# Kamino666/Video-Captioning-Transformer

Measured on AMD Instinct MI355X. Metric: video-caption train samples/sec (whole node), higher is better.
Workload: dtype bf16; 1 GPU; configs[1]: 2 enc + 2 dec layers d=512 ff=2048 H=8 V=30522, synthetic (256,12,512) features -> 20-token captions per GPU, fwd+bwd+Adam, dropout 0.3, SCE alpha 0.5; global_batch=256, per_gpu_batch=256, seq_len=20, frames=12, parallelism=dp1, executor=list

## Files before the change

video-captioning-transformer_amd/csrc/vct_layer_ss.hip:

```cpp
#include "vct_layer_ss_core.h"

namespace vct {

template <bool CROSS, int MT>
__global__ __launch_bounds__(SS_NT, SS_NW / 4) void layer_ss_fwd_kernel(const SsLayerP p) {
  extern __shared__ __attribute__((aligned(16))) unsigned char smem[];
  const int tid0 = threadIdx.x, lane0 = tid0 & 63;
  const int wave = __builtin_amdgcn_readfirstlane(tid0 >> 6);
  const int b = blockIdx.x, L = p.L;
  const long grow0 = (long)b * L;
  bf16_t* R0 = reinterpret_cast<bf16_t*>(smem + SS_R0);
  bf16_t* R1A = reinterpret_cast<bf16_t*>(smem + SS_R1A);
  bf16_t* R1B = reinterpret_cast<bf16_t*>(smem + SS_R1B);
  bf16_t* R1C = reinterpret_cast<bf16_t*>(smem + SS_R1C);
  bf16_t* RMp = reinterpret_cast<bf16_t*>(smem + SS_RM);
  float* red = reinterpret_cast<float*>(smem + SS_RED);
  float* b1s = reinterpret_cast<float*>(smem + SS_B1);

  WStream ws;
  ws.p = p.wpk + (long)wave * SS_WSTR + lane0 * 8;
  ws.last = ws.p + (long)(p.nchunks - 1) * SS_CHUNK;
  bf16x8 b0[SS_TPW][2], b1[SS_TPW][2];
  ws_fetch(ws, b0);
  ws_fetch(ws, b1);

  if constexpr (CROSS) global_to_panel(RMp, SS_PSTR, p.Lm, 16, p.mem, SS_D, (long)b * p.Lm, tid0);
  const unsigned long long padmask = ss_padmask(p, b, lane0);
  if (!CROSS && p.pro == 1) {
    const int T = L - 1, li = lane0 & 15, lg = lane0 >> 4;
    for (int v = tid0; v < MT * 16 * (SS_D / 8); v += SS_NT) {
      const int r = v / (SS_D / 8), c = (v % (SS_D / 8)) * 8;
      BV8s val;
      if (r < T) {
        const long g = ((long)b * T + r) * SS_D + c;
        if (p.feats_f32) {
          const float4 f0 = *reinterpret_cast<const float4*>(reinterpret_cast<const float*>(p.feats) + g);
          const float4 f1 = *reinterpret_cast<const float4*>(reinterpret_cast<const float*>(p.feats) + g + 4);
          val.e[0] = f2bf(f0.x); val.e[1] = f2bf(f0.y); val.e[2] = f2bf(f0.z); val.e[3] = f2bf(f0.w);
          val.e[4] = f2bf(f1.x); val.e[5] = f2bf(f1.y); val.e[6] = f2bf(f1.z); val.e[7] = f2bf(f1.w);
          if (p.x_in != nullptr) *reinterpret_cast<BV8s*>(p.x_in + g) = val;
        } else {
          val = *reinterpret_cast<const BV8s*>(reinterpret_cast<const bf16_t*>(p.feats) + g);
        }
      } else {
#pragma unroll
        for (int j = 0; j < 8; j++) val.e[j] = 0;
      }
      *reinterpret_cast<BV8s*>(R1A + r * SS_PSTR + c) = val;
    }
    float4 bu[SS_TPW];
    load_bias4(bu, p.b_u, wave * SS_CPW, lg);
    ss_barrier();
    f32x4 au[MT][SS_TPW];
    acc_zero<MT>(au);
    wave_gemm<MT>(au, R1A + li * SS_PSTR + lg * 8, SS_PSTR, 0, 8, ws, b0, b1);
    const float invT = 1.0f / (float)T;
#pragma unroll
    for (int t = 0; t < SS_TPW; t++) {
      const int col = wave * SS_CPW + t * 16 + lg * 4;
      float cs[4] = {0.0f, 0.0f, 0.0f, 0.0f};
      const float bb[4] = {bu[t].x, bu[t].y, bu[t].z, bu[t].w};
#pragma unroll
      for (int m = 0; m < MT; m++) {
        const int fr = m * 16 + li;
        const bool valid = fr < T;
        const float4 pe4 = *reinterpret_cast<const float4*>(p.pe + (long)min(fr + 1, T) * SS_D + col);
        const float pp[4] = {pe4.x, pe4.y, pe4.z, pe4.w};
        BV4 z;
#pragma unroll
        for (int r = 0; r < 4; r++) {
          const float u = bf2f(f2bf(au[m][t][r] + bb[r]));
          cs[r] += valid ? u : 0.0f;
          z.e[r] = valid ? f2bf(u + pp[r]) : (bf16_t)0;
        }
        if (fr + 1 < MT * 16) *reinterpret_cast<BV4*>(R0 + (fr + 1) * SS_PSTR + col) = z;
      }
#pragma unroll
      for (int r = 0; r < 4; r++) cs[r] = red16_sum(cs[r]);
      if (li == 0) {
        const float4 pe0 = *reinterpret_cast<const float4*>(p.pe + col);
        BV4 z;
        z.e[0] = f2bf(cs[0] * invT + pe0.x); z.e[1] = f2bf(cs[1] * invT + pe0.y); z.e[2] = f2bf(cs[2] * invT + pe0.z); z.e[3] = f2bf(cs[3] * invT + pe0.w);
        *reinterpret_cast<BV4*>(R0 + col) = z;
      }
    }
    ss_barrier();
    panel_to_global<SS_D>(R0, SS_PSTR, L, p.x, SS_D, grow0, 0, tid0);
  } else if (CROSS && p.pro == 2) {
    const Dropout dre = make_dropout(p.seed, p.site_emb, p.p_drop);
    for (int v = tid0; v < MT * 16 * (SS_D / 8); v += SS_NT) {
      const int r = v / (SS_D / 8), c = (v % (SS_D / 8)) * 8;
      BV8s val;
      if (r < L) {
        const long id = p.emb_ids[(long)b * p.emb_ids_bs + r];
        const float* tr = p.emb_table + id * SS_D + c;
        const float* pr = p.emb_pos + (long)r * SS_D + c;
        const float4 t0 = *reinterpret_cast<const float4*>(tr), t1 = *reinterpret_cast<const float4*>(tr + 4);
        const float4 q0 = *reinterpret_cast<const float4*>(pr), q1 = *reinterpret_cast<const float4*>(pr + 4);
        float dm[8];
        drop_mults<8>(dre, (uint32_t)(grow0 + r) * (uint32_t)SS_D + (uint32_t)c, dm);
        val.e[0] = f2bf((t0.x + q0.x) * dm[0]); val.e[1] = f2bf((t0.y + q0.y) * dm[1]); val.e[2] = f2bf((t0.z + q0.z) * dm[2]);
        val.e[3] = f2bf((t0.w + q0.w) * dm[3]); val.e[4] = f2bf((t1.x + q1.x) * dm[4]); val.e[5] = f2bf((t1.y + q1.y) * dm[5]);
        val.e[6] = f2bf((t1.z + q1.z) * dm[6]); val.e[7] = f2bf((t1.w + q1.w) * dm[7]);
        *reinterpret_cast<BV8s*>(p.x + (grow0 + r) * SS_D + c) = val;
      } else {
#pragma unroll
        for (int j = 0; j < 8; j++) val.e[j] = 0;
      }
      *reinterpret_cast<BV8s*>(R0 + r * SS_PSTR + c) = val;
    }
  } else {
    global_to_panel(R0, SS_PSTR, L, MT * 16, p.x, SS_D, grow0, tid0);
  }
  constexpr int SS_WPH = SS_NW / SS_H;
  const int head = wave / SS_WPH, qt0 = wave % SS_WPH, hd0 = head * SS_HD;
  bf16_t* FIN = CROSS ? R0 : R1B;
  bf16_t* HP0 = CROSS ? R1B : R0;
  bf16_t* HP1 = R1C;
  bf16_t* FP = R1A;
  bf16_t* YP = R0;
  bf16_t* Y2P = R1C;

  typedef const __attribute__((address_space(4))) SsLayerP* KargP;
  const KargP kp = (KargP)__builtin_amdgcn_kernarg_segment_ptr();
  for (int l = 0; l < p.nl; l++) {
    int tid = tid0;
    asm volatile("" : "+v"(tid));
    const int lane = tid & 63, li = lane & 15, lg = lane >> 4;
    const int aoff = li * SS_PSTR + lg * 8;
    const int ecol = wave * SS_CPW + lg * 4;
    const __attribute__((address_space(4))) SsLayerW& w = kp->lw[l];
    auto nrm = [](const __attribute__((address_space(4))) SsNorm& n) { return SsNorm{n.g, n.b, n.y, n.mean, n.rstd}; };
    const bool fin = p.last && l == p.nl - 1;
    for (int v = tid; v < (p.ff >> 2); v += SS_NT) reinterpret_cast<float4*>(b1s)[v] = reinterpret_cast<const float4*>(w.b1)[v];
    SS_STAMP(0);
    ss_barrier();
    SS_STAMP(1);

    f32x4 acc[MT][SS_TPW];
    float4 bv[SS_TPW];
    for (int nb = 0; nb < 3; nb++) {
      load_bias4(bv, w.b_qkv, nb * 512 + wave * SS_CPW, lg);
      acc_zero<MT>(acc);
      wave_gemm<MT>(acc, R0 + aoff, SS_PSTR, 0, 8, ws, b0, b1);
      epi_store<MT>(acc, bv, R1A, SS_QSTR, nb * 512 + wave * SS_CPW, li, lg);
    }
    BV4 res[MT][SS_TPW];
#pragma unroll
    for (int m = 0; m < MT; m++)
#pragma unroll
      for (int t = 0; t < SS_TPW; t++) res[m][t] = *reinterpret_cast<const BV4*>(R0 + (m * 16 + li) * SS_PSTR + ecol + t * 16);
    SS_STAMP(2);
    ss_barrier();
    SS_STAMP(3);
    panel_to_global<3 * SS_D>(R1A, SS_QSTR, L, w.qkv, 3 * SS_D, grow0, 0, tid);
    SS_STAMP(4);
    {
      const Dropout dr = make_dropout(p.seed, w.site_sa, p.p_drop);
      ss_attn_wave(R1A + hd0, SS_QSTR, R1A + SS_D + hd0, R1A + 2 * SS_D + hd0, SS_QSTR, L, L, p.causal, padmask, dr,
                   b * SS_H + head, R0 + hd0, lane, qt0, SS_WPH);
    }
    SS_STAMP(5);
    ss_barrier();
    SS_STAMP(6);
    panel_to_global<SS_D>(R0, SS_PSTR, L, w.o, SS_D, grow0, 0, tid);
    SS_STAMP(7);
    {
      load_bias4(bv, w.b_o, wave * SS_CPW, lg);
      acc_zero<MT>(acc);
      wave_gemm<MT>(acc, R0 + aoff, SS_PSTR, 0, 8, ws, b0, b1);
      SS_STAMP(8);
      const Dropout dr = make_dropout(p.seed, w.site_n1, p.p_drop);
      epi_ln<MT>(acc, bv, res, nrm(w.n1), nullptr, dr, grow0, L, R1A, R1B, nullptr, red, wave, li, lg);
      SS_STAMP(9);
    }
    ss_barrier();
    panel_to_global<SS_D>(R1A, SS_PSTR, L, w.a, SS_D, grow0, 0, tid);
    panel_to_global<SS_D>(R1B, SS_PSTR, L, w.n1.y, SS_D, grow0, 0, tid);
    SS_STAMP(10);

    if constexpr (CROSS) {
      const int Lm = p.Lm;
      load_bias4(bv, w.b_cq, wave * SS_CPW, lg);
      acc_zero<MT>(acc);
      wave_gemm<MT>(acc, R1B + aoff, SS_PSTR, 0, 8, ws, b0, b1);
      epi_store<MT>(acc, bv, R1C, SS_PSTR, wave * SS_CPW, li, lg);
      SS_STAMP(11);
      for (int nb = 0; nb < 2; nb++) {
        f32x4 acm[1][SS_TPW];
        load_bias4(bv, w.b_ckv, nb * 512 + wave * SS_CPW, lg);
        acc_zero<1>(acm);
        wave_gemm<1>(acm, RMp + aoff, SS_PSTR, 0, 8, ws, b0, b1);
        epi_store<1>(acm, bv, R0, SS_KVSTR, nb * 512 + wave * SS_CPW, li, lg);
      }
      SS_STAMP(12);
      ss_barrier();
      panel_to_global<SS_D>(R1C, SS_PSTR, L, w.cq, SS_D, grow0, 0, tid);
      panel_to_global<2 * SS_D>(R0, SS_KVSTR, Lm, w.ckv, 2 * SS_D, (long)b * Lm, 0, tid);
      SS_STAMP(13);
      {
        const Dropout dr = make_dropout(p.seed, w.site_ca, p.p_drop);
        ss_attn_wave(R1C + hd0, SS_PSTR, R0 + hd0, R0 + SS_D + hd0, SS_KVSTR, L, Lm, 0, 0ull, dr, b * SS_H + head,
                     R1A + hd0, lane, qt0, SS_WPH);
      }
      SS_STAMP(14);
      ss_barrier();
      panel_to_global<SS_D>(R1A, SS_PSTR, L, w.co, SS_D, grow0, 0, tid);
      SS_STAMP(15);
      {
#pragma unroll
        for (int m = 0; m < MT; m++)
#pragma unroll
          for (int t = 0; t < SS_TPW; t++) res[m][t] = *reinterpret_cast<const BV4*>(R1B + (m * 16 + li) * SS_PSTR + ecol + t * 16);
        load_bias4(bv, w.b_co, wave * SS_CPW, lg);
        acc_zero<MT>(acc);
        wave_gemm<MT>(acc, R1A + aoff, SS_PSTR, 0, 8, ws, b0, b1);
        SS_STAMP(16);
        const Dropout dr = make_dropout(p.seed, w.site_n2, p.p_drop);
        epi_ln<MT>(acc, bv, res, nrm(w.n2), nullptr, dr, grow0, L, R1C, R0, nullptr, red, wave, li, lg);
        SS_STAMP(17);
      }
      ss_barrier();
      panel_to_global<SS_D>(R1C, SS_PSTR, L, w.ca, SS_D, grow0, 0, tid);
      panel_to_global<SS_D>(R0, SS_PSTR, L, w.n2.y, SS_D, grow0, 0, tid);
      SS_STAMP(18);
    }

    f32x4 facc[MT][SS_TPW];
    BV4 hpk[MT][SS_TPW];
    acc_zero<MT>(facc);
    const Dropout drf = make_dropout(p.seed, w.site_ff, p.p_drop);
    const int nj = p.ff >> 9;
    auto ffn_pre = [&](const int j) {
#pragma unroll
      for (int m = 0; m < MT; m++)
#pragma unroll
        for (int t = 0; t < SS_TPW; t++) {
          const int row = m * 16 + li, col = j * 512 + ecol + t * 16;
          const float4 bb = *reinterpret_cast<const float4*>(b1s + col);
          BV4 pv;
          pv.e[0] = f2bf(acc[m][t][0] + bb.x); pv.e[1] = f2bf(acc[m][t][1] + bb.y);
          pv.e[2] = f2bf(acc[m][t][2] + bb.z); pv.e[3] = f2bf(acc[m][t][3] + bb.w);
          hpk[m][t] = pv;
#if SS_STREAM_STORES
          if (row < L) store_stream8(w.hpre + (grow0 + row) * p.ff + col, __builtin_bit_cast(stream_u32x2, pv));
#else
          if (row < L) *reinterpret_cast<BV4*>(w.hpre + (grow0 + row) * p.ff + col) = pv;
#endif
        }
    };
    auto ffn_tile = [&](const int j, auto K) {
      constexpr int k = decltype(K)::value;
      if constexpr (k < MT * SS_TPW) {
        constexpr int m = k / SS_TPW, t = k % SS_TPW;
        const int row = m * 16 + li;
        const int col = j * 512 + ecol + t * 16;
        float dm[4];
        drop_mults<4>(drf, (uint32_t)(grow0 + row) * (uint32_t)p.ff + (uint32_t)col, dm);
        const vf2 x0 = {bf2f(hpk[m][t].e[0]), bf2f(hpk[m][t].e[1])}, x1 = {bf2f(hpk[m][t].e[2]), bf2f(hpk[m][t].e[3])};
        const vf2 a0 = act_fast_f2(p.act, x0) * vf2{dm[0], dm[1]}, a1 = act_fast_f2(p.act, x1) * vf2{dm[2], dm[3]};
        BV4 hv;
        hv.e[0] = f2bf(a0[0]); hv.e[1] = f2bf(a0[1]); hv.e[2] = f2bf(a1[0]); hv.e[3] = f2bf(a1[1]);
        *reinterpret_cast<BV4*>(((j & 1) ? HP1 : HP0) + row * SS_PSTR + ecol + t * 16) = hv;
      }
    };
    load_bias4(bv, w.b2, wave * SS_CPW, lg);
    acc_zero<MT>(acc);
    wave_gemm<MT>(acc, FIN + aoff, SS_PSTR, 0, 8, ws, b0, b1);
    ffn_pre(0);
    SS_STAMP(20);
    for (int j = 0; j < nj; j++) {
      if (j + 1 < nj) {
        acc_zero<MT>(acc);
        wave_gemm8_cb<MT>(acc, FIN + aoff, SS_PSTR, ws, b0, b1, [&](auto K) { ffn_tile(j, K); });
      } else {
        static_for<MT * SS_TPW>([&](auto K) { ffn_tile(j, K); });
      }
      SS_STAMP(21 + 4 * j);
      ss_barrier();
      bf16_t* HP = (j & 1) ? HP1 : HP0;
      panel_to_global<SS_D>(HP, SS_PSTR, L, w.h, p.ff, grow0, j * 512, tid);
      SS_STAMP(22 + 4 * j);
      wave_gemm<MT>(facc, HP + aoff, SS_PSTR, 0, 8, ws, b0, b1);
      if (j + 1 < nj) ffn_pre(j + 1);
      SS_STAMP(23 + 4 * j);
    }
    {
#pragma unroll
      for (int m = 0; m < MT; m++)
#pragma unroll
        for (int t = 0; t < SS_TPW; t++) res[m][t] = *reinterpret_cast<const BV4*>(FIN + (m * 16 + li) * SS_PSTR + ecol + t * 16);
      ss_barrier();
      const Dropout dr = make_dropout(p.seed, w.site_n3, p.p_drop);
      const SsNorm nfl = p.nf;
      epi_ln<MT>(facc, bv, res, nrm(w.n3), fin ? &nfl : nullptr, dr, grow0, L, FP, YP, Y2P, red, wave, li, lg);
      SS_STAMP(40);
    }
    ss_barrier();
    panel_to_global<SS_D>(FP, SS_PSTR, L, w.f, SS_D, grow0, 0, tid);
    panel_to_global<SS_D>(YP, SS_PSTR, L, w.n3.y, SS_D, grow0, 0, tid);
    if (fin) panel_to_global<SS_D>(Y2P, SS_PSTR, L, p.nf.y, SS_D, grow0, 0, tid);
    SS_STAMP(41);
  }
}

constexpr int SS_PACK_MAX = 48;
struct SsPackSeg { const bf16_t* w; long ldw; int nchunks; int dst_chunk; int tr; };
struct SsPackP { SsPackSeg seg[SS_PACK_MAX]; int nseg; bf16_t* dst; };

__global__ __launch_bounds__(256) void ss_pack_kernel(const SsPackP p) {
  const int sg = blockIdx.y;
  if (sg >= p.nseg) return;
  const SsPackSeg s = p.seg[sg];
  const long v = (long)blockIdx.x * 256 + threadIdx.x;
  if (v >= (long)s.nchunks * (SS_CHUNK / 8)) return;
  constexpr int FPW = 2 * SS_TPW;
  const int lane = (int)(v & 63), frag = (int)((v >> 6) % FPW), w = (int)((v >> 6) / FPW % SS_NW);
  const long c = v >> 12;
  const int t = frag >> 1, ks = frag & 1;
  const int n = w * SS_CPW + t * 16 + (lane & 15);
  const long k = c * 64 + ks * 32 + (lane >> 4) * 8;
  BV8s val;
  if (s.tr) {
#pragma unroll
    for (int j = 0; j < 8; j++) val.e[j] = s.w[(k + j) * s.ldw + n];
  } else {
    val = *reinterpret_cast<const BV8s*>(s.w + (long)n * s.ldw + k);
  }
  *reinterpret_cast<BV8s*>(p.dst + ((long)s.dst_chunk + c) * SS_CHUNK + (v & 4095) * 8) = val;
}

}
using namespace vct;

extern "C" int vct_layer_ss_supported(int dtype, int d, int H, int ff, int L, int Lm) {
  if (dtype != VCT_BF16 || d != SS_D || H != SS_H) return 0;
  if (ff < 512 || (ff % 512) != 0 || ff > SS_FF_MAX) return 0;
  if (L < 1 || L > 32) return 0;
  if (Lm < 0 || Lm > 16) return 0;
  return 1;
}

extern "C" int64_t vct_layer_ss_stream_chunks(int ff, int cross) {
  return (int64_t)8 * (4 + (cross ? 4 : 0) + 2 * (ff / 512));
}

extern "C" int vct_ss_pack(const vct_ss_pack_seg* segs, int nseg, void* dst, void* stream) {
  if (segs == nullptr || dst == nullptr || nseg < 1) return VCT_E_ARG;
  if (((uintptr_t)dst & 15)) return VCT_E_ALIGN;
  hipStream_t st = (hipStream_t)stream;
  for (int base = 0; base < nseg; base += SS_PACK_MAX) {
    SsPackP p;
    p.nseg = nseg - base < SS_PACK_MAX ? nseg - base : SS_PACK_MAX;
    p.dst = reinterpret_cast<bf16_t*>(dst);
    int maxch = 0;
    for (int i = 0; i < p.nseg; i++) {
      const vct_ss_pack_seg& s = segs[base + i];
      if (s.w == nullptr || s.nchunks < 1 || s.dst_chunk < 0) return VCT_E_ARG;
      if ((s.ldw % 8) || ((uintptr_t)s.w & 15)) return VCT_E_ALIGN;
      p.seg[i].w = reinterpret_cast<const bf16_t*>(s.w); p.seg[i].ldw = s.ldw; p.seg[i].nchunks = s.nchunks; p.seg[i].dst_chunk = (int)s.dst_chunk; p.seg[i].tr = s.transposed != 0;
      maxch = s.nchunks > maxch ? s.nchunks : maxch;
    }
    for (int i = p.nseg; i < SS_PACK_MAX; i++) p.seg[i] = SsPackSeg{nullptr, 0, 0, 0, 0};
    const dim3 grid((unsigned)((long)maxch * (SS_CHUNK / 8) / 256), p.nseg);
    vct::launch(ss_pack_kernel, grid, dim3(256), 0, st, p);
    VCT_CHECK_LAUNCH();
  }
  return VCT_OK;
}

extern "C" int vct_layer_ss_fwd(const vct_layer_ss_desc* layers, int n_layers, void* stream) {
  if (layers == nullptr || n_layers < 1) return VCT_E_ARG;
  const vct_layer_ss_desc* q = layers;
  const int cross = q->mem != nullptr;
  if (!vct_layer_ss_supported(q->dtype, q->d, q->H, q->ff, q->L, cross ? q->Lm : 0) || q->B < 1) return VCT_E_SHAPE;
  if (cross && q->Lm < 1) return VCT_E_SHAPE;
  const int64_t per_layer = vct_layer_ss_stream_chunks(q->ff, cross);
  const int pro = q->pro;
  if (pro < 0 || pro > 2 || (pro == 1 && cross) || (pro == 2 && !cross)) return VCT_E_ARG;
  if (pro == 1 && (!q->feats || !q->b_unify || !q->pe_rows || q->L < 2 || (q->feats_dtype != VCT_F32 && q->feats_dtype != VCT_BF16) ||
                   (((uintptr_t)q->feats | (uintptr_t)q->x_in | (uintptr_t)q->b_unify | (uintptr_t)q->pe_rows) & 15)))
    return VCT_E_ARG;
  if (pro == 2 && (!q->emb_ids || !q->emb_table || !q->emb_pos || (((uintptr_t)q->emb_table | (uintptr_t)q->emb_pos) & 15))) return VCT_E_ARG;
  const int64_t pro_chunks = pro == 1 ? 8 : 0;
  if (!q->x || q->key_pad_shift < 0 || (q->key_pad != nullptr && q->key_pad_shift >= q->L)) return q->x ? VCT_E_SHAPE : VCT_E_ARG;
  auto norm_ok = [](const vct_ss_norm& n) { return n.gamma && n.beta && n.y && n.mean && n.rstd; };
  auto cvt = [](const vct_ss_norm& n) { return SsNorm{n.gamma, n.beta, reinterpret_cast<bf16_t*>(n.y), n.mean, n.rstd}; };
  for (int l = 0; l < n_layers; l++) {
    const vct_layer_ss_desc& d = layers[l];
    if (d.dtype != q->dtype || d.B != q->B || d.L != q->L || d.Lm != q->Lm || d.d != q->d || d.H != q->H || d.ff != q->ff || d.act != q->act ||
        d.causal != q->causal || d.key_pad_shift != q->key_pad_shift || d.mem != q->mem || d.key_pad != q->key_pad || d.key_ids != q->key_ids ||
        d.key_ids_bs != q->key_ids_bs || d.pad_id != q->pad_id || d.seed != q->seed || d.p_drop != q->p_drop)
      return VCT_E_ARG;
    if (d.nchunks != per_layer) return VCT_E_SHAPE;
    if (!d.wpk || (const char*)d.wpk != (const char*)q->wpk + (size_t)(l * per_layer + (l > 0 ? pro_chunks : 0)) * SS_CHUNK * 2) return VCT_E_ARG;
    if (l > 0 && d.pro != 0) return VCT_E_ARG;
    if (d.last && l != n_layers - 1) return VCT_E_ARG;
    if (!d.b_qkv || !d.b_o || !d.qkv || !d.o || !d.a || !d.b1 || !d.b2 || !d.hpre || !d.h || !d.f) return VCT_E_ARG;
    if (!norm_ok(d.n1) || !norm_ok(d.n3) || (d.last && !norm_ok(d.nf))) return VCT_E_ARG;
    if (cross && (!d.b_cq || !d.b_ckv || !d.b_co || !d.cq || !d.ckv || !d.co || !d.ca || !norm_ok(d.n2))) return VCT_E_ARG;
    const uintptr_t al = (uintptr_t)d.wpk | (uintptr_t)d.x | (uintptr_t)d.mem | (uintptr_t)d.qkv | (uintptr_t)d.o | (uintptr_t)d.a |
                         (uintptr_t)d.cq | (uintptr_t)d.ckv | (uintptr_t)d.co | (uintptr_t)d.ca | (uintptr_t)d.hpre | (uintptr_t)d.h |
                         (uintptr_t)d.f | (uintptr_t)d.n1.y | (uintptr_t)d.n2.y | (uintptr_t)d.n3.y | (uintptr_t)d.nf.y |
                         (uintptr_t)d.b_qkv | (uintptr_t)d.b_o | (uintptr_t)d.b_cq | (uintptr_t)d.b_ckv | (uintptr_t)d.b_co |
                         (uintptr_t)d.b1 | (uintptr_t)d.b2;
    if (al & 15) return VCT_E_ALIGN;
  }
  hipStream_t st = (hipStream_t)stream;
  const int one = q->L <= 16 ? 1 : 0, which = cross * 2 + one;
  static vct::DynLdsOptIn optin[4];
  const void* fn = which == 0 ? (const void*)layer_ss_fwd_kernel<false, 2> : which == 1 ? (const void*)layer_ss_fwd_kernel<false, 1>
                 : which == 2 ? (const void*)layer_ss_fwd_kernel<true, 2> : (const void*)layer_ss_fwd_kernel<true, 1>;
  if (hipError_t e = optin[which].ensure(fn, SS_LDS); e != hipSuccess) return (int)e;
  for (int base = 0; base < n_layers; base += SS_MAXL) {
    const int nl = n_layers - base < SS_MAXL ? n_layers - base : SS_MAXL;
    SsLayerP p;
    memset(&p, 0, sizeof(p));
    p.B = q->B; p.L = q->L; p.Lm = cross ? q->Lm : 0; p.ff = q->ff; p.act = q->act; p.causal = q->causal; p.nl = nl;
    p.last = layers[base + nl - 1].last;
    p.wpk = reinterpret_cast<const bf16_t*>(layers[base].wpk); p.nchunks = (int)(per_layer * nl + (base == 0 ? pro_chunks : 0));
    p.x = const_cast<bf16_t*>(reinterpret_cast<const bf16_t*>(base == 0 ? q->x : layers[base - 1].n3.y));
    p.pro = base == 0 ? pro : 0;
    p.feats = q->feats; p.feats_f32 = q->feats_dtype == VCT_F32; p.x_in = reinterpret_cast<bf16_t*>(q->x_in); p.b_u = q->b_unify; p.pe = q->pe_rows;
    p.emb_ids = q->emb_ids; p.emb_ids_bs = q->emb_ids_bs; p.emb_table = q->emb_table; p.emb_pos = q->emb_pos; p.site_emb = q->site_emb;
    p.mem = reinterpret_cast<const bf16_t*>(q->mem);
    p.nf = cvt(layers[base + nl - 1].nf);
    p.key_pad = q->key_pad; p.key_pad_shift = q->key_pad_shift; p.key_ids = q->key_ids; p.key_ids_bs = q->key_ids_bs; p.pad_id = q->pad_id;
    p.seed = q->seed; p.p_drop = q->p_drop;
    for (int l = 0; l < nl; l++) {
      const vct_layer_ss_desc& d = layers[base + l];
      SsLayerW& w = p.lw[l];
      w.b_qkv = d.b_qkv; w.b_o = d.b_o;
      w.qkv = reinterpret_cast<bf16_t*>(d.qkv); w.o = reinterpret_cast<bf16_t*>(d.o); w.a = reinterpret_cast<bf16_t*>(d.a);
      w.n1 = cvt(d.n1); w.n2 = cvt(d.n2); w.n3 = cvt(d.n3);
      w.b_cq = d.b_cq; w.b_ckv = d.b_ckv; w.b_co = d.b_co;
      w.cq = reinterpret_cast<bf16_t*>(d.cq); w.ckv = reinterpret_cast<bf16_t*>(d.ckv); w.co = reinterpret_cast<bf16_t*>(d.co);
      w.ca = reinterpret_cast<bf16_t*>(d.ca);
      w.b1 = d.b1; w.b2 = d.b2;
      w.hpre = reinterpret_cast<bf16_t*>(d.hpre); w.h = reinterpret_cast<bf16_t*>(d.h); w.f = reinterpret_cast<bf16_t*>(d.f);
      w.site_sa = d.site_sa; w.site_n1 = d.site_n1; w.site_ca = d.site_ca; w.site_n2 = d.site_n2; w.site_ff = d.site_ff; w.site_n3 = d.site_n3;
    }
#ifdef SS_STAMPS
    p.dbg = g_ss_dbg;
#endif
    if (which == 0) vct::launch(layer_ss_fwd_kernel<false, 2>, dim3(p.B), dim3(SS_NT), SS_LDS, st, p);
    else if (which == 1) vct::launch(layer_ss_fwd_kernel<false, 1>, dim3(p.B), dim3(SS_NT), SS_LDS, st, p);
    else if (which == 2) vct::launch(layer_ss_fwd_kernel<true, 2>, dim3(p.B), dim3(SS_NT), SS_LDS, st, p);
    else vct::launch(layer_ss_fwd_kernel<true, 1>, dim3(p.B), dim3(SS_NT), SS_LDS, st, p);
    VCT_CHECK_LAUNCH();
  }
  return VCT_OK;
}
```

video-captioning-transformer_amd/csrc/vct_layer_ss_core.h:

```cpp
#pragma once
#include <cstring>
#include "vct_attn_core.h"

namespace vct {

constexpr int SS_D = 512, SS_H = 8, SS_HD = 64;
constexpr int SS_NW = 8, SS_NT = SS_NW * 64;
constexpr int SS_TPW = 32 / SS_NW;
constexpr int SS_CPW = SS_TPW * 16;
constexpr int SS_WSTR = SS_TPW * 2 * 512;
constexpr int SS_PSTR = SS_D + 8;
constexpr int SS_SLOT = 32 * SS_PSTR * 2;
constexpr int SS_QSTR = 3 * SS_D + 8;
constexpr int SS_KVSTR = 2 * SS_D + 8;
constexpr int SS_R0 = 0, SS_R1A = SS_SLOT, SS_R1B = 2 * SS_SLOT, SS_R1C = 3 * SS_SLOT;
constexpr int SS_RM = 4 * SS_SLOT;
constexpr int SS_RED = SS_RM + 16 * SS_PSTR * 2;
constexpr int SS_B1 = SS_RED + 2 * SS_NW * 32 * 4;
constexpr int SS_FF_MAX = 2048;
constexpr int SS_LDS = SS_B1 + SS_FF_MAX * 4;
constexpr long SS_CHUNK = 32768;
static_assert(SS_LDS <= 160 * 1024, "LDS budget");
static_assert(32 * SS_QSTR * 2 <= 3 * SS_SLOT && 16 * SS_KVSTR * 2 <= SS_SLOT, "panel slots");

struct SsNorm { const float* g; const float* b; bf16_t* y; float* mean; float* rstd; };

constexpr int SS_MAXL = 4;

struct SsLayerW {
  const float* b_qkv; const float* b_o;
  bf16_t* qkv; bf16_t* o; bf16_t* a;
  SsNorm n1;
  const float* b_cq; const float* b_ckv; const float* b_co;
  bf16_t* cq; bf16_t* ckv; bf16_t* co; bf16_t* ca;
  SsNorm n2;
  const float* b1; const float* b2;
  bf16_t* hpre; bf16_t* h; bf16_t* f;
  SsNorm n3;
  uint32_t site_sa, site_n1, site_ca, site_n2, site_ff, site_n3;
};

struct SsLayerP {
  int B, L, Lm;
  int ff, act, last, causal, nl;
  const bf16_t* wpk; int nchunks;
  bf16_t* x;
  const bf16_t* mem;
  int pro;
  const void* feats; int feats_f32; bf16_t* x_in; const float* b_u; const float* pe;
  const int64_t* emb_ids; long emb_ids_bs; const float* emb_table; const float* emb_pos; uint32_t site_emb;
  SsNorm nf;
  const uint8_t* key_pad; int key_pad_shift;
  const int64_t* key_ids; long key_ids_bs; long pad_id;
  const uint32_t* seed; float p_drop;
  SsLayerW lw[SS_MAXL];
#ifdef SS_STAMPS
  unsigned long long* dbg;
#endif
};
#ifdef SS_STAMPS
#ifdef SS_STAMPS_ALLWAVES
#define SS_STAMP(i) do { if ((tid & 63) == 0) p.dbg[((long)blockIdx.x * 8 + (tid >> 6)) * 64 + (i)] = __builtin_readcyclecounter(); } while (0)
#else
#define SS_STAMP(i) do { if (tid == 0) p.dbg[(long)blockIdx.x * 64 + (i)] = __builtin_readcyclecounter(); } while (0)
#endif
#else
#define SS_STAMP(i) do { } while (0)
#endif

__device__ __forceinline__ void ss_barrier() {
  asm volatile("s_waitcnt lgkmcnt(0)" ::: "memory");
  __builtin_amdgcn_s_barrier();
  asm volatile("" ::: "memory");
}

struct WStream {
  const bf16_t* p;
  const bf16_t* last;
};
__device__ __forceinline__ void ws_fetch(WStream& ws, bf16x8 (&dst)[SS_TPW][2]) {
#pragma unroll
  for (int t = 0; t < SS_TPW; t++)
#pragma unroll
    for (int s = 0; s < 2; s++) dst[t][s] = *reinterpret_cast<const bf16x8*>(ws.p + (t * 2 + s) * 512);
  ws.p = (ws.p + SS_CHUNK <= ws.last) ? ws.p + SS_CHUNK : ws.last;
}

template <int MT>
__device__ __forceinline__ void gemm_step(f32x4 (&acc)[MT][SS_TPW], const bf16_t* a, const int astr, const int kc, const bf16x8 (&b)[SS_TPW][2]) {
  bf16x8 af[MT][2];
#pragma unroll
  for (int m = 0; m < MT; m++)
#pragma unroll
    for (int s = 0; s < 2; s++) af[m][s] = *reinterpret_cast<const bf16x8*>(a + m * 16 * astr + kc * 64 + s * 32);
#pragma unroll
  for (int s = 0; s < 2; s++)
#pragma unroll
    for (int m = 0; m < MT; m++)
#pragma unroll
      for (int t = 0; t < SS_TPW; t++) acc[m][t] = __builtin_amdgcn_mfma_f32_16x16x32_bf16(b[t][s], af[m][s], acc[m][t], 0, 0, 0);
}
template <int MT>
__device__ __forceinline__ void wave_gemm(f32x4 (&acc)[MT][SS_TPW], const bf16_t* a, const int astr, const int kc0, const int nch, WStream& ws,
                                          bf16x8 (&b0)[SS_TPW][2], bf16x8 (&b1)[SS_TPW][2]) {
  for (int c = 0; c < nch; c += 2) {
    gemm_step<MT>(acc, a, astr, kc0 + c, b0);
    ws_fetch(ws, b0);
    gemm_step<MT>(acc, a, astr, kc0 + c + 1, b1);
    ws_fetch(ws, b1);
  }
}
template <int MT, class F>
__device__ __forceinline__ void wave_gemm8_cb(f32x4 (&acc)[MT][SS_TPW], const bf16_t* a, const int astr, WStream& ws, bf16x8 (&b0)[SS_TPW][2],
                                              bf16x8 (&b1)[SS_TPW][2], F&& cb) {
  static_for<4>([&](auto I) {
    constexpr int i = decltype(I)::value;
    cb(std::integral_constant<int, 2 * i>{});
    gemm_step<MT>(acc, a, astr, 2 * i, b0);
    ws_fetch(ws, b0);
    cb(std::integral_constant<int, 2 * i + 1>{});
    gemm_step<MT>(acc, a, astr, 2 * i + 1, b1);
    ws_fetch(ws, b1);
  });
}

template <int MT> __device__ __forceinline__ void acc_zero(f32x4 (&acc)[MT][SS_TPW]) {
#pragma unroll
  for (int m = 0; m < MT; m++)
#pragma unroll
    for (int t = 0; t < SS_TPW; t++) acc[m][t] = f32x4{0, 0, 0, 0};
}

__device__ __forceinline__ void load_bias4(float4 (&bv)[SS_TPW], const float* bias, const int col0, const int lg) {
#pragma unroll
  for (int t = 0; t < SS_TPW; t++) bv[t] = *reinterpret_cast<const float4*>(bias + col0 + t * 16 + lg * 4);
}

struct alignas(8) BV4 { bf16_t e[4]; };
struct alignas(16) BV8s { bf16_t e[8]; };
#ifndef SS_STREAM_STORES
#define SS_STREAM_STORES 0
#endif

template <int NCOLS>
__device__ __forceinline__ void panel_to_global(const bf16_t* panel, const int pstr, const int rows, bf16_t* g, const long ld,
                                                const long row0, const int col0, const int tid) {
  constexpr int vpr = NCOLS / 8;
  const int total = rows * vpr;
  for (int v = tid; v < total; v += SS_NT) {
    const int r = v / vpr, c = (v - r * vpr) * 8;
#if SS_STREAM_STORES
    store_stream16(g + (row0 + r) * ld + col0 + c, *reinterpret_cast<const stream_u32x4*>(panel + r * pstr + c));
#else
    *reinterpret_cast<BV8s*>(g + (row0 + r) * ld + col0 + c) = *reinterpret_cast<const BV8s*>(panel + r * pstr + c);
#endif
  }
}
__device__ __forceinline__ void global_to_panel(bf16_t* panel, const int pstr, const int L, const int alloc, const bf16_t* g, const long ld,
                                                const long row0, const int tid) {
  constexpr int vpr = SS_D / 8;
  for (int v = tid; v < alloc * vpr; v += SS_NT) {
    const int r = v / vpr, c = (v - r * vpr) * 8;
    BV8s val;
    if (r < L) val = *reinterpret_cast<const BV8s*>(g + (row0 + r) * ld + c);
    else {
#pragma unroll
      for (int j = 0; j < 8; j++) val.e[j] = 0;
    }
    *reinterpret_cast<BV8s*>(panel + r * pstr + c) = val;
  }
}

__device__ __forceinline__ void load_gb(float4 (&gm)[SS_TPW], float4 (&bt)[SS_TPW], const SsNorm& n, const int ecol) {
#pragma unroll
  for (int t = 0; t < SS_TPW; t++) {
    gm[t] = *reinterpret_cast<const float4*>(n.g + ecol + t * 16);
    bt[t] = *reinterpret_cast<const float4*>(n.b + ecol + t * 16);
  }
}

template <int MT>
__device__ __forceinline__ void epi_store(const f32x4 (&acc)[MT][SS_TPW], const float4 (&bv)[SS_TPW], bf16_t* panel, const int pstr, const int pcol0,
                                          const int li, const int lg) {
#pragma unroll
  for (int m = 0; m < MT; m++)
#pragma unroll
    for (int t = 0; t < SS_TPW; t++) {
      BV4 o;
      o.e[0] = f2bf(acc[m][t][0] + bv[t].x); o.e[1] = f2bf(acc[m][t][1] + bv[t].y);
      o.e[2] = f2bf(acc[m][t][2] + bv[t].z); o.e[3] = f2bf(acc[m][t][3] + bv[t].w);
      *reinterpret_cast<BV4*>(panel + (m * 16 + li) * pstr + pcol0 + t * 16 + lg * 4) = o;
    }
}

template <int MT>
__device__ __forceinline__ void epi_ln(f32x4 (&acc)[MT][SS_TPW], const float4 (&bv)[SS_TPW], const BV4 (&res)[MT][SS_TPW], const SsNorm& n, const SsNorm* n2,
                                       const Dropout& dr, const long grow0, const int L, bf16_t* AP, bf16_t* YP, bf16_t* Y2P, float* red,
                                       const int wave, const int li_in, const int lg_in) {
  int li = li_in, lg = lg_in;
  asm volatile("" : "+v"(li), "+v"(lg));
  const int colw = wave * SS_CPW + lg * 4;
  float4 gm[SS_TPW], bt[SS_TPW];
  load_gb(gm, bt, n, colw);
  float part[MT];
#pragma unroll
  for (int m = 0; m < MT; m++) {
    part[m] = 0.0f;
    const uint32_t grow = (uint32_t)(grow0 + m * 16 + li);
#pragma unroll
    for (int t = 0; t < SS_TPW; t++) {
      const float bb[4] = {bv[t].x, bv[t].y, bv[t].z, bv[t].w};
      float dm[4];
      drop_mults<4>(dr, grow * (uint32_t)SS_D + (uint32_t)(colw + t * 16), dm);
      BV4 av;
#pragma unroll
      for (int r = 0; r < 4; r++) {
        av.e[r] = f2bf(acc[m][t][r] + bb[r]);
        const float s = bf2f(av.e[r]) * dm[r] + bf2f(res[m][t].e[r]);
        acc[m][t][r] = s;
        part[m] += s;
      }
      *reinterpret_cast<BV4*>(AP + (m * 16 + li) * SS_PSTR + colw + t * 16) = av;
    }
    part[m] = red4_sum(part[m]);
  }
  float* red0 = red;
  float* red1 = red + SS_NW * 32;
  auto stats = [&](float (&mean)[MT], float (&rstd)[MT]) {
    if (lg == 0) {
#pragma unroll
      for (int m = 0; m < MT; m++) red0[wave * 32 + m * 16 + li] = part[m];
    }
    ss_barrier();
    float sq[MT];
#pragma unroll
    for (int m = 0; m < MT; m++) {
      float s = 0.0f;
#pragma unroll
      for (int w = 0; w < SS_NW; w++) s += red0[w * 32 + m * 16 + li];
      mean[m] = s * (1.0f / (float)SS_D);
      sq[m] = 0.0f;
#pragma unroll
      for (int t = 0; t < SS_TPW; t++)
#pragma unroll
        for (int r = 0; r < 4; r++) { const float c = acc[m][t][r] - mean[m]; sq[m] += c * c; }
      sq[m] = red4_sum(sq[m]);
    }
    if (lg == 0) {
#pragma unroll
      for (int m = 0; m < MT; m++) red1[wave * 32 + m * 16 + li] = sq[m];
    }
    ss_barrier();
#pragma unroll
    for (int m = 0; m < MT; m++) {
      float v = 0.0f;
#pragma unroll
      for (int w = 0; w < SS_NW; w++) v += red1[w * 32 + m * 16 + li];
      rstd[m] = 1.0f / sqrtf(v * (1.0f / (float)SS_D) + 1e-5f);
    }
  };
  float mean[MT], rstd[MT];
  stats(mean, rstd);
  if (wave == 0 && lg == 0) {
#pragma unroll
    for (int m = 0; m < MT; m++)
      if (m * 16 + li < L) { n.mean[grow0 + m * 16 + li] = mean[m]; n.rstd[grow0 + m * 16 + li] = rstd[m]; }
  }
#pragma unroll
  for (int m = 0; m < MT; m++) {
    part[m] = 0.0f;
#pragma unroll
    for (int t = 0; t < SS_TPW; t++) {
      const float gg[4] = {gm[t].x, gm[t].y, gm[t].z, gm[t].w}, be[4] = {bt[t].x, bt[t].y, bt[t].z, bt[t].w};
      BV4 yv;
#pragma unroll
      for (int r = 0; r < 4; r++) {
        yv.e[r] = f2bf((acc[m][t][r] - mean[m]) * rstd[m] * gg[r] + be[r]);
        acc[m][t][r] = bf2f(yv.e[r]);
        part[m] += acc[m][t][r];
      }
      *reinterpret_cast<BV4*>(YP + (m * 16 + li) * SS_PSTR + colw + t * 16) = yv;
    }
    part[m] = red4_sum(part[m]);
  }
  if (n2 != nullptr) {
#pragma unroll
    for (int t = 0; t < SS_TPW; t++) {
      gm[t] = *reinterpret_cast<const float4*>(n2->g + colw + t * 16);
      bt[t] = *reinterpret_cast<const float4*>(n2->b + colw + t * 16);
    }
    stats(mean, rstd);
    if (wave == 0 && lg == 0) {
#pragma unroll
      for (int m = 0; m < MT; m++)
        if (m * 16 + li < L) { n2->mean[grow0 + m * 16 + li] = mean[m]; n2->rstd[grow0 + m * 16 + li] = rstd[m]; }
    }
#pragma unroll
    for (int m = 0; m < MT; m++)
#pragma unroll
      for (int t = 0; t < SS_TPW; t++) {
        const float gg[4] = {gm[t].x, gm[t].y, gm[t].z, gm[t].w}, be[4] = {bt[t].x, bt[t].y, bt[t].z, bt[t].w};
        BV4 yv;
#pragma unroll
        for (int r = 0; r < 4; r++) yv.e[r] = f2bf((acc[m][t][r] - mean[m]) * rstd[m] * gg[r] + be[r]);
        *reinterpret_cast<BV4*>(Y2P + (m * 16 + li) * SS_PSTR + colw + t * 16) = yv;
      }
  }
}

__device__ __forceinline__ bf16x8 ss_frag_rowk(const bf16_t* p, const int str, const int row_base, const int ks, const int lane) {
  return *reinterpret_cast<const bf16x8*>(p + (row_base + (lane & 15)) * str + ks * 32 + (lane >> 4) * 8);
}
__device__ __forceinline__ bf16x8 ss_frag_colk(const bf16_t* p, const int str, const int r0, const int r1, const int col_base, const int lane) {
  const int i = lane & 15, g = lane >> 4;
  const s16x4 lo = lds_tr16(p + (r0 + g * 4 + (i >> 2)) * str + col_base + (i & 3) * 4);
  const s16x4 hi = lds_tr16(p + (r1 + g * 4 + (i >> 2)) * str + col_base + (i & 3) * 4);
  const s16x8 v = {lo[0], lo[1], lo[2], lo[3], hi[0], hi[1], hi[2], hi[3]};
  return __builtin_bit_cast(bf16x8, v);
}
__device__ __forceinline__ void ss_attn_wave(const bf16_t* Qp, const int strq, const bf16_t* Kp, const bf16_t* Vp, const int strkv, const int Lq,
                                             const int Lk, const int causal, const unsigned long long padmask, const Dropout& dr, const int bh,
                                             bf16_t* OPh, const int lane, const int qt0, const int qstep) {
  const int i = lane & 15, g = lane >> 4;
  const int LQT = (Lq + 15) >> 4, LKT = (Lk + 15) >> 4;
  const float scale = 0.125f;
  for (int qt = qt0; qt < LQT; qt += qstep) {
    f32x4 st[2];
    const int qq = qt * 16 + i;
#pragma unroll
    for (int t = 0; t < 2; t++) {
      st[t] = f32x4{0, 0, 0, 0};
      if (t < LKT) {
#pragma unroll
        for (int ks = 0; ks < 2; ks++)
          st[t] = __builtin_amdgcn_mfma_f32_16x16x32_bf16(ss_frag_rowk(Kp, strkv, t * 16, ks, lane), ss_frag_rowk(Qp, strq, qt * 16, ks, lane),
                                                          st[t], 0, 0, 0);
      }
#pragma unroll
      for (int r = 0; r < 4; r++) {
        const int kk = t * 16 + g * 4 + r;
        const bool masked = kk >= Lk || (causal && kk > qq) || ((padmask >> kk) & 1ull);
        st[t][r] = (t < LKT && !masked) ? st[t][r] * scale : -INFINITY;
      }
    }
    float m = -INFINITY;
#pragma unroll
    for (int t = 0; t < 2; t++)
#pragma unroll
      for (int r = 0; r < 4; r++) m = fmaxf(m, st[t][r]);
    m = red4_max(m);
    if (m == -INFINITY) m = 0.0f;
    float l = 0.0f;
#pragma unroll
    for (int t = 0; t < 2; t++) {
      if (t < LKT) {
#pragma unroll
        for (int r = 0; r < 4; r++) { st[t][r] = __expf(st[t][r] - m); l += st[t][r]; }
      } else {
        st[t] = f32x4{0, 0, 0, 0};
      }
    }
    l = red4_sum(l);
    const float inv = l > 0.0f ? 1.0f / l : 0.0f;
#pragma unroll
    for (int t = 0; t < 2; t++)
      if (t < LKT) {
#pragma unroll
        for (int r = 0; r < 4; r++) {
          const int kk = t * 16 + g * 4 + r;
          st[t][r] *= inv * drop_mult(dr, (uint32_t)((bh * Lq + qq) * Lk + kk));
        }
      }
    const bf16x8 pa = pack_p(st[0], st[1]);
    const int r1 = LKT > 1 ? 16 : 0;
#pragma unroll
    for (int dt = 0; dt < 4; dt++) {
      f32x4 ot = __builtin_amdgcn_mfma_f32_16x16x32_bf16(ss_frag_colk(Vp, strkv, 0, r1, dt * 16, lane), pa, f32x4{0, 0, 0, 0}, 0, 0, 0);
      BV4 o;
#pragma unroll
      for (int r = 0; r < 4; r++) o.e[r] = f2bf(ot[r]);
      *reinterpret_cast<BV4*>(OPh + (qt * 16 + i) * SS_PSTR + dt * 16 + g * 4) = o;
    }
  }
}

template <class P> __device__ __forceinline__ unsigned long long ss_padmask(const P& p, const int b, const int lane) {
  if (p.key_ids != nullptr) {
    const long id = p.key_ids[(long)b * p.key_ids_bs + min(lane, p.L - 1)];
    return __ballot(lane < p.L && id == p.pad_id);
  }
  if (p.key_pad == nullptr) return 0ull;
  const int w = p.L - p.key_pad_shift;
  const int j = min(max(lane - p.key_pad_shift, 0), w - 1);
  const uint8_t v = p.key_pad[(long)b * w + j];
  return __ballot(lane >= p.key_pad_shift && lane < p.L && v != 0);
}


}
```

Baseline: 124,000 samples/s.

## Interleave activation panel stores to global into subsequent GEMM k-steps

The standalone LDS-panel-to-global copies (qkv, o, a, x1, cq, ckv, co, ca, x2, h, and the next layer's input y) that used to run between barriers are now sliced across the 8 k-chunks of the next wave GEMM through a callback, so the global stores overlap with MFMA work instead of stalling between phases. epi_ln gains a mode that holds the pre-norm output in registers and writes it to LDS only after the first reduction barrier, which is needed because that LDS region is still being copied out by the overlapped stores. The per-layer n3.y store is deferred into the next layer's first QKV GEMM. This adds register pressure and depends on correct buffer lifetimes across barriers.

```diff
diff --git a/video-captioning-transformer_amd/csrc/vct_layer_ss.hip b/video-captioning-transformer_amd/csrc/vct_layer_ss.hip
--- a/video-captioning-transformer_amd/csrc/vct_layer_ss.hip
+++ b/video-captioning-transformer_amd/csrc/vct_layer_ss.hip
@@ -132,6 +132,7 @@
     const __attribute__((address_space(4))) SsLayerW& w = kp->lw[l];
     auto nrm = [](const __attribute__((address_space(4))) SsNorm& n) { return SsNorm{n.g, n.b, n.y, n.mean, n.rstd}; };
     const bool fin = p.last && l == p.nl - 1;
+    constexpr int IT1 = ss_copy_its(MT * 16, SS_D), IT3 = ss_copy_its(MT * 16, 3 * SS_D), ITKV = ss_copy_its(16, 2 * SS_D);
     for (int v = tid; v < (p.ff >> 2); v += SS_NT) reinterpret_cast<float4*>(b1s)[v] = reinterpret_cast<const float4*>(w.b1)[v];
     SS_STAMP(0);
     ss_barrier();
@@ -142,7 +143,14 @@
     for (int nb = 0; nb < 3; nb++) {
       load_bias4(bv, w.b_qkv, nb * 512 + wave * SS_CPW, lg);
       acc_zero<MT>(acc);
-      wave_gemm<MT>(acc, R0 + aoff, SS_PSTR, 0, 8, ws, b0, b1);
+      if (nb == 0 && l > 0) {
+        bf16_t* const gy = kp->lw[l - 1].n3.y;
+        wave_gemm8_cb<MT>(acc, R0 + aoff, SS_PSTR, ws, b0, b1, [&](auto K) {
+          panel_to_global_slice<SS_D, decltype(K)::value, 0, IT1, IT1>(R0, SS_PSTR, L, gy, SS_D, grow0, 0, tid);
+        });
+      } else {
+        wave_gemm<MT>(acc, R0 + aoff, SS_PSTR, 0, 8, ws, b0, b1);
+      }
       epi_store<MT>(acc, bv, R1A, SS_QSTR, nb * 512 + wave * SS_CPW, li, lg);
     }
     BV4 res[MT][SS_TPW];
@@ -153,8 +161,6 @@
     SS_STAMP(2);
     ss_barrier();
     SS_STAMP(3);
-    panel_to_global<3 * SS_D>(R1A, SS_QSTR, L, w.qkv, 3 * SS_D, grow0, 0, tid);
-    SS_STAMP(4);
     {
       const Dropout dr = make_dropout(p.seed, w.site_sa, p.p_drop);
       ss_attn_wave(R1A + hd0, SS_QSTR, R1A + SS_D + hd0, R1A + 2 * SS_D + hd0, SS_QSTR, L, L, p.causal, padmask, dr,
@@ -163,27 +169,33 @@
     SS_STAMP(5);
     ss_barrier();
     SS_STAMP(6);
-    panel_to_global<SS_D>(R0, SS_PSTR, L, w.o, SS_D, grow0, 0, tid);
-    SS_STAMP(7);
     {
       load_bias4(bv, w.b_o, wave * SS_CPW, lg);
       acc_zero<MT>(acc);
-      wave_gemm<MT>(acc, R0 + aoff, SS_PSTR, 0, 8, ws, b0, b1);
+      bf16_t* const gqkv = w.qkv; bf16_t* const go = w.o;
+      wave_gemm8_cb<MT>(acc, R0 + aoff, SS_PSTR, ws, b0, b1, [&](auto K) {
+        constexpr int k = decltype(K)::value;
+        panel_to_global_slice<3 * SS_D, k, 0, IT3, IT3 + IT1>(R1A, SS_QSTR, L, gqkv, 3 * SS_D, grow0, 0, tid);
+        panel_to_global_slice<SS_D, k, IT3, IT1, IT3 + IT1>(R0, SS_PSTR, L, go, SS_D, grow0, 0, tid);
+      });
       SS_STAMP(8);
       const Dropout dr = make_dropout(p.seed, w.site_n1, p.p_drop);
-      epi_ln<MT>(acc, bv, res, nrm(w.n1), nullptr, dr, grow0, L, R1A, R1B, nullptr, red, wave, li, lg);
+      epi_ln<MT, true>(acc, bv, res, nrm(w.n1), SsNorm{}, false, dr, grow0, L, R1A, R1B, nullptr, red, wave, li, lg);
       SS_STAMP(9);
     }
     ss_barrier();
-    panel_to_global<SS_D>(R1A, SS_PSTR, L, w.a, SS_D, grow0, 0, tid);
-    panel_to_global<SS_D>(R1B, SS_PSTR, L, w.n1.y, SS_D, grow0, 0, tid);
     SS_STAMP(10);
+    auto copy_a_x1 = [&, ga = w.a, gx1 = w.n1.y](auto K) {
+      constexpr int k = decltype(K)::value;
+      panel_to_global_slice<SS_D, k, 0, IT1, 2 * IT1>(R1A, SS_PSTR, L, ga, SS_D, grow0, 0, tid);
+      panel_to_global_slice<SS_D, k, IT1, IT1, 2 * IT1>(R1B, SS_PSTR, L, gx1, SS_D, grow0, 0, tid);
+    };
 
     if constexpr (CROSS) {
       const int Lm = p.Lm;
       load_bias4(bv, w.b_cq, wave * SS_CPW, lg);
       acc_zero<MT>(acc);
-      wave_gemm<MT>(acc, R1B + aoff, SS_PSTR, 0, 8, ws, b0, b1);
+      wave_gemm8_cb<MT>(acc, R1B + aoff, SS_PSTR, ws, b0, b1, copy_a_x1);
       epi_store<MT>(acc, bv, R1C, SS_PSTR, wave * SS_CPW, li, lg);
       SS_STAMP(11);
       for (int nb = 0; nb < 2; nb++) {
@@ -195,8 +207,6 @@
       }
       SS_STAMP(12);
       ss_barrier();
-      panel_to_global<SS_D>(R1C, SS_PSTR, L, w.cq, SS_D, grow0, 0, tid);
-      panel_to_global<2 * SS_D>(R0, SS_KVSTR, Lm, w.ckv, 2 * SS_D, (long)b * Lm, 0, tid);
       SS_STAMP(13);
       {
         const Dropout dr = make_dropout(p.seed, w.site_ca, p.p_drop);
@@ -205,7 +215,6 @@
       }
       SS_STAMP(14);
       ss_barrier();
-      panel_to_global<SS_D>(R1A, SS_PSTR, L, w.co, SS_D, grow0, 0, tid);
       SS_STAMP(15);
       {
 #pragma unroll
@@ -214,15 +223,19 @@
           for (int t = 0; t < SS_TPW; t++) res[m][t] = *reinterpret_cast<const BV4*>(R1B + (m * 16 + li) * SS_PSTR + ecol + t * 16);
         load_bias4(bv, w.b_co, wave * SS_CPW, lg);
         acc_zero<MT>(acc);
-        wave_gemm<MT>(acc, R1A + aoff, SS_PSTR, 0, 8, ws, b0, b1);
+        bf16_t* const gcq = w.cq; bf16_t* const gckv = w.ckv; bf16_t* const gco = w.co;
+        wave_gemm8_cb<MT>(acc, R1A + aoff, SS_PSTR, ws, b0, b1, [&](auto K) {
+          constexpr int k = decltype(K)::value, tot = 2 * IT1 + ITKV;
+          panel_to_global_slice<SS_D, k, 0, IT1, tot>(R1C, SS_PSTR, L, gcq, SS_D, grow0, 0, tid);
+          panel_to_global_slice<2 * SS_D, k, IT1, ITKV, tot>(R0, SS_KVSTR, Lm, gckv, 2 * SS_D, (long)b * Lm, 0, tid);
+          panel_to_global_slice<SS_D, k, IT1 + ITKV, IT1, tot>(R1A, SS_PSTR, L, gco, SS_D, grow0, 0, tid);
+        });
         SS_STAMP(16);
         const Dropout dr = make_dropout(p.seed, w.site_n2, p.p_drop);
-        epi_ln<MT>(acc, bv, res, nrm(w.n2), nullptr, dr, grow0, L, R1C, R0, nullptr, red, wave, li, lg);
+        epi_ln<MT, true>(acc, bv, res, nrm(w.n2), SsNorm{}, false, dr, grow0, L, R1C, R0, nullptr, red, wave, li, lg);
         SS_STAMP(17);
       }
       ss_barrier();
-      panel_to_global<SS_D>(R1C, SS_PSTR, L, w.ca, SS_D, grow0, 0, tid);
-      panel_to_global<SS_D>(R0, SS_PSTR, L, w.n2.y, SS_D, grow0, 0, tid);
       SS_STAMP(18);
     }
 
@@ -231,6 +244,8 @@
     acc_zero<MT>(facc);
     const Dropout drf = make_dropout(p.seed, w.site_ff, p.p_drop);
     const int nj = p.ff >> 9;
+    bf16_t* const gh = w.h;
+    const long ff = p.ff;
     auto ffn_pre = [&](const int j) {
 #pragma unroll
       for (int m = 0; m < MT; m++)
@@ -266,7 +281,16 @@
     };
     load_bias4(bv, w.b2, wave * SS_CPW, lg);
     acc_zero<MT>(acc);
-    wave_gemm<MT>(acc, FIN + aoff, SS_PSTR, 0, 8, ws, b0, b1);
+    if constexpr (CROSS) {
+      bf16_t* const gca = w.ca; bf16_t* const gx2 = w.n2.y;
+      wave_gemm8_cb<MT>(acc, FIN + aoff, SS_PSTR, ws, b0, b1, [&](auto K) {
+        constexpr int k = decltype(K)::value;
+        panel_to_global_slice<SS_D, k, 0, IT1, 2 * IT1>(R1C, SS_PSTR, L, gca, SS_D, grow0, 0, tid);
+        panel_to_global_slice<SS_D, k, IT1, IT1, 2 * IT1>(R0, SS_PSTR, L, gx2, SS_D, grow0, 0, tid);
+      });
+    } else {
+      wave_gemm8_cb<MT>(acc, FIN + aoff, SS_PSTR, ws, b0, b1, copy_a_x1);
+    }
     ffn_pre(0);
     SS_STAMP(20);
     for (int j = 0; j < nj; j++) {
@@ -279,9 +303,10 @@
       SS_STAMP(21 + 4 * j);
       ss_barrier();
       bf16_t* HP = (j & 1) ? HP1 : HP0;
-      panel_to_global<SS_D>(HP, SS_PSTR, L, w.h, p.ff, grow0, j * 512, tid);
       SS_STAMP(22 + 4 * j);
-      wave_gemm<MT>(facc, HP + aoff, SS_PSTR, 0, 8, ws, b0, b1);
+      wave_gemm8_cb<MT>(facc, HP + aoff, SS_PSTR, ws, b0, b1, [&](auto K) {
+        panel_to_global_slice<SS_D, decltype(K)::value, 0, IT1, IT1>(HP, SS_PSTR, L, gh, ff, grow0, j * 512, tid);
+      });
       if (j + 1 < nj) ffn_pre(j + 1);
       SS_STAMP(23 + 4 * j);
     }
@@ -292,13 +317,12 @@
         for (int t = 0; t < SS_TPW; t++) res[m][t] = *reinterpret_cast<const BV4*>(FIN + (m * 16 + li) * SS_PSTR + ecol + t * 16);
       ss_barrier();
       const Dropout dr = make_dropout(p.seed, w.site_n3, p.p_drop);
-      const SsNorm nfl = p.nf;
-      epi_ln<MT>(facc, bv, res, nrm(w.n3), fin ? &nfl : nullptr, dr, grow0, L, FP, YP, Y2P, red, wave, li, lg);
+      epi_ln<MT>(facc, bv, res, nrm(w.n3), nrm(kp->nf), fin, dr, grow0, L, FP, YP, Y2P, red, wave, li, lg);
       SS_STAMP(40);
     }
     ss_barrier();
     panel_to_global<SS_D>(FP, SS_PSTR, L, w.f, SS_D, grow0, 0, tid);
-    panel_to_global<SS_D>(YP, SS_PSTR, L, w.n3.y, SS_D, grow0, 0, tid);
+    if (l + 1 == p.nl) panel_to_global<SS_D>(YP, SS_PSTR, L, w.n3.y, SS_D, grow0, 0, tid);
     if (fin) panel_to_global<SS_D>(Y2P, SS_PSTR, L, p.nf.y, SS_D, grow0, 0, tid);
     SS_STAMP(41);
   }
diff --git a/video-captioning-transformer_amd/csrc/vct_layer_ss_core.h b/video-captioning-transformer_amd/csrc/vct_layer_ss_core.h
--- a/video-captioning-transformer_amd/csrc/vct_layer_ss_core.h
+++ b/video-captioning-transformer_amd/csrc/vct_layer_ss_core.h
@@ -156,6 +156,29 @@
 #endif
   }
 }
+__host__ __device__ constexpr int ss_copy_its(const int rows_alloc, const int ncols) { return (rows_alloc * (ncols / 8) + SS_NT - 1) / SS_NT; }
+template <int NCOLS, int K, int OFF, int NIT, int TOT>
+__device__ __forceinline__ void panel_to_global_slice(const bf16_t* panel, const int pstr, const int rows, bf16_t* g, const long ld,
+                                                      const long row0, const int col0, const int tid) {
+  static_assert(TOT >= OFF + NIT && (TOT - 1) * 8 / TOT <= 7, "copy list");
+  constexpr int vpr = NCOLS / 8;
+  static_for<NIT>([&](auto I) {
+    constexpr int it = decltype(I)::value;
+    if constexpr ((OFF + it) * 8 / TOT == K) {
+      int tv = tid;
+      asm volatile("" : "+v"(tv));
+      const int v = tv + it * SS_NT;
+      if (v < rows * vpr) {
+        const int r = v / vpr, c = (v - r * vpr) * 8;
+#if SS_STREAM_STORES
+        store_stream16(g + (row0 + r) * ld + col0 + c, *reinterpret_cast<const stream_u32x4*>(panel + r * pstr + c));
+#else
+        *reinterpret_cast<BV8s*>(g + (row0 + r) * ld + col0 + c) = *reinterpret_cast<const BV8s*>(panel + r * pstr + c);
+#endif
+      }
+    }
+  });
+}
 __device__ __forceinline__ void global_to_panel(bf16_t* panel, const int pstr, const int L, const int alloc, const bf16_t* g, const long ld,
                                                 const long row0, const int tid) {
   constexpr int vpr = SS_D / 8;
@@ -193,9 +216,9 @@
     }
 }
 
-template <int MT>
-__device__ __forceinline__ void epi_ln(f32x4 (&acc)[MT][SS_TPW], const float4 (&bv)[SS_TPW], const BV4 (&res)[MT][SS_TPW], const SsNorm& n, const SsNorm* n2,
-                                       const Dropout& dr, const long grow0, const int L, bf16_t* AP, bf16_t* YP, bf16_t* Y2P, float* red,
+template <int MT, bool AP_LATE = false>
+__device__ __forceinline__ void epi_ln(f32x4 (&acc)[MT][SS_TPW], const float4 (&bv)[SS_TPW], const BV4 (&res)[MT][SS_TPW], const SsNorm n, const SsNorm n2,
+                                       const bool has2, const Dropout& dr, const long grow0, const int L, bf16_t* AP, bf16_t* YP, bf16_t* Y2P, float* red,
                                        const int wave, const int li_in, const int lg_in) {
   int li = li_in, lg = lg_in;
   asm volatile("" : "+v"(li), "+v"(lg));
@@ -203,6 +226,7 @@
   float4 gm[SS_TPW], bt[SS_TPW];
   load_gb(gm, bt, n, colw);
   float part[MT];
+  BV4 avl[AP_LATE ? MT : 1][SS_TPW];
 #pragma unroll
   for (int m = 0; m < MT; m++) {
     part[m] = 0.0f;
@@ -220,18 +244,25 @@
         acc[m][t][r] = s;
         part[m] += s;
       }
-      *reinterpret_cast<BV4*>(AP + (m * 16 + li) * SS_PSTR + colw + t * 16) = av;
+      if constexpr (AP_LATE) avl[m][t] = av;
+      else *reinterpret_cast<BV4*>(AP + (m * 16 + li) * SS_PSTR + colw + t * 16) = av;
     }
     part[m] = red4_sum(part[m]);
   }
   float* red0 = red;
   float* red1 = red + SS_NW * 32;
-  auto stats = [&](float (&mean)[MT], float (&rstd)[MT]) {
+  auto stats = [&](float (&mean)[MT], float (&rstd)[MT], auto FIRST) {
     if (lg == 0) {
 #pragma unroll
       for (int m = 0; m < MT; m++) red0[wave * 32 + m * 16 + li] = part[m];
     }
     ss_barrier();
+    if constexpr (AP_LATE && decltype(FIRST)::value) {
+#pragma unroll
+      for (int m = 0; m < MT; m++)
+#pragma unroll
+        for (int t = 0; t < SS_TPW; t++) *reinterpret_cast<BV4*>(AP + (m * 16 + li) * SS_PSTR + colw + t * 16) = avl[m][t];
+    }
     float sq[MT];
 #pragma unroll
     for (int m = 0; m < MT; m++) {
@@ -260,7 +291,7 @@
     }
   };
   float mean[MT], rstd[MT];
-  stats(mean, rstd);
+  stats(mean, rstd, std::true_type{});
   if (wave == 0 && lg == 0) {
 #pragma unroll
     for (int m = 0; m < MT; m++)
@@ -283,17 +314,17 @@
     }
     part[m] = red4_sum(part[m]);
   }
-  if (n2 != nullptr) {
+  if (has2) {
 #pragma unroll
     for (int t = 0; t < SS_TPW; t++) {
-      gm[t] = *reinterpret_cast<const float4*>(n2->g + colw + t * 16);
-      bt[t] = *reinterpret_cast<const float4*>(n2->b + colw + t * 16);
-    }
-    stats(mean, rstd);
+      gm[t] = *reinterpret_cast<const float4*>(n2.g + colw + t * 16);
+      bt[t] = *reinterpret_cast<const float4*>(n2.b + colw + t * 16);
+    }
+    stats(mean, rstd, std::false_type{});
     if (wave == 0 && lg == 0) {
 #pragma unroll
       for (int m = 0; m < MT; m++)
-        if (m * 16 + li < L) { n2->mean[grow0 + m * 16 + li] = mean[m]; n2->rstd[grow0 + m * 16 + li] = rstd[m]; }
+        if (m * 16 + li < L) { n2.mean[grow0 + m * 16 + li] = mean[m]; n2.rstd[grow0 + m * 16 + li] = rstd[m]; }
     }
 #pragma unroll
     for (int m = 0; m < MT; m++)
```

New measurement: 125,600 samples/s, median of 6. +1.3%, better.
